# mirage/decompress

Measured on AMD Instinct MI355X. Metric: MiB/s inflate over N zlib streams (uncompressed bytes / wall second), higher is better.
Workload: dtype u8; 1 GPU; C2: 4096 x 256 KiB zlib streams per GPU, dynamic Huffman (libz level 6; even streams = slices of the reference's test/corpus, odd = order-2 Markov ASCII text, 64 symbols, seed 0xC2 + i, SURVEY 8(d)), Zl.Inf.Ns semantics, one stream per pair of wavefronts (decoder + copier); streams_per_gpu=4096, stream_bytes=262144, unique_streams=4096

## Files before the change

decompress_amd/csrc/inflate_wave.hip:

```cpp
#include <stdlib.h>
#include <string.h>
#include "inflate_util.hpp"

namespace md {
namespace wv {

constexpr uint32_t S = 264;
constexpr uint32_t SMIN = 48;
constexpr uint32_t KMAX = 64;
#ifndef MD_EMIT_SPLIT
#define MD_EMIT_SPLIT 1
#endif
#if defined(MD_DEBUG_KNOWN_BOUNDS)
#undef MD_EMIT_SPLIT
#define MD_EMIT_SPLIT 0
#endif
#ifndef MD_SPLIT_B
#define MD_SPLIT_B 4
#endif
#ifndef MD_RUNIN_NUM
#define MD_RUNIN_NUM 3
#define MD_RUNIN_DEN 2
#endif
constexpr uint32_t RUNIN_NUM = MD_RUNIN_NUM, RUNIN_DEN = MD_RUNIN_DEN;
constexpr uint32_t PASSES = 5;
constexpr uint32_t PASS_BITS = 1600, PASSES_MAX = 16;
#ifndef MD_RMAX
#define MD_RMAX 576
#endif
#ifndef MD_STAGE
#define MD_STAGE 5248
#endif
#ifndef MD_PAIR_OCC
#define MD_PAIR_OCC 5
#endif
constexpr uint32_t RMAX = MD_RMAX;
constexpr uint32_t STAGE = MD_STAGE;
constexpr uint32_t WIN_WORDS = 544;

constexpr uint32_t kLitSize = 852, kDistSize = 592;
constexpr uint32_t kLitRootMax = 512;
constexpr uint32_t kLitSubB = 0;
constexpr uint32_t kDistB = kLitSize - kLitRootMax;
constexpr uint32_t kLitB = kDistB + kDistSize;
constexpr uint32_t kStopEobI = kLitB + kLitRootMax;
constexpr uint32_t kStopBadI = kStopEobI + 2;
constexpr uint32_t kLutWords = kStopBadI + 2;
constexpr uint32_t kTbMask = 0xffe00000u;
constexpr uint32_t kLoopy = 0x100u;
static_assert(kDistB % 2 == 0 && kLitB % 2 == 0 && kStopEobI % 2 == 0 && kLutWords == 1448, "even table bases");
constexpr uint32_t kStEob = 100, kStTrunc = 101;
constexpr uint32_t kCountMatch = 1u << 20;
constexpr uint32_t kNearBit = 0x8000u;

struct Mail {
  uint32_t emitted;
  uint32_t copied;
  uint32_t kind;
  uint32_t total;
  uint32_t x;
  uint32_t stuck;
  uint32_t a, b;
};
constexpr uint32_t kJobRound = 0, kJobStored = 1, kJobQuit = 2, kJobEmit = 3;
constexpr uint32_t kHxUni = 4 * 64;
struct Smem {
  uint32_t win[WIN_WORDS];
  uint32_t lut[kLutWords];
  uint32_t mrec[RMAX];
  uint16_t mpos[RMAX];
  alignas(16) uint8_t stage[STAGE + 16];
  uint16_t list[RMAX];
  Mail mail;
};
struct HScratch {
  uint8_t lens[384];
  uint16_t work[320];
  uint32_t ctr;
};
#if MD_RMAX == 576 && MD_STAGE == 5248
static_assert(sizeof(Smem) <= 17920, "9 streams (18 wavefronts) per CU: 160 KiB / 9, in whole 512-byte units");
#endif
static_assert(RMAX % 64 == 0 && STAGE % 16 == 0 && RMAX * 2 >= (kHxUni + 6) * 4, "record rows, staging chunks, the emit job's words in `list`");
constexpr uint32_t kHScratchAt = 1136;
static_assert(kHScratchAt >= 4 + 572 + 8 && kHScratchAt % 16 == 0 && kHScratchAt + sizeof(HScratch) <= WIN_WORDS * 4, "header scratch lives behind the header's bits");
typedef MD_LDS Smem lds_smem;
typedef MD_LDS HScratch lds_hscratch;
__device__ __forceinline__ lds_hscratch *hscratch_of(lds_smem *sm) {
  return reinterpret_cast<lds_hscratch *>(reinterpret_cast<lds_u8 *>(sm->win) + kHScratchAt);
}

#ifdef MD_DEBUG_KNOWN_BOUNDS
constexpr uint32_t KB_ROUNDS = 512;
__device__ uint4 *g_kb_buf;
__device__ int g_kb_mode;
#endif
__device__ __forceinline__ uint32_t mk_entry(uint32_t n, uint32_t xb, uint32_t val8, uint32_t nbits, uint32_t tb) {
  return n | (xb << 5) | (val8 << 9) | (nbits << 17) | (tb << 21);
}
__device__ __forceinline__ uint32_t e_n(uint32_t e) { return e & 31; }
__device__ __forceinline__ uint32_t e_xb(uint32_t e) { return (e >> 5) & 15; }
__device__ __forceinline__ uint32_t e_val(uint32_t e) { return (e >> 9) & 255; }
__device__ __forceinline__ uint32_t e_tb(uint32_t e) { return e >> 21; }
__device__ __forceinline__ bool e_link(uint32_t e) { return e_tb(e) < kLitB && e_tb(e) != kDistB; }
__device__ __forceinline__ uint32_t e_root(uint32_t lroot) { return mk_entry(0, 0, 0, lroot, kLitB); }
__device__ __forceinline__ uint32_t lit_leaf(uint32_t sym, uint32_t codelen, uint32_t lroot, uint32_t droot) {
  if (sym < 256) return mk_entry(codelen, 0, sym, lroot, kLitB);
  if (sym == 256) return mk_entry(codelen, 0, 0, 0, kStopEobI);
  const uint32_t l = (sym - 257) & 31;
  const uint32_t xb = (l >= 8 && l < 28) ? (l - 4) >> 2 : 0;
  const uint32_t base3 = l < 8 ? l : l < 28 ? (4 + (l & 3)) << xb : l == 28 ? 255 : 0;
  return mk_entry(codelen + xb, xb, base3, droot, kDistB);
}
__device__ __forceinline__ uint32_t dist_leaf(uint32_t dv, uint32_t codelen, uint32_t lroot) {
  dv &= 31;
  if (dv >= 30) return mk_entry(codelen, 0, 0, 0, kStopBadI);
  const uint32_t xb = dv >= 4 ? (dv - 2) >> 1 : 0;
  const uint32_t m = dv < 4 ? dv : ((dv & 1) | 2);
  return mk_entry(codelen + xb, xb, m, lroot, kLitB);
}
__device__ __forceinline__ uint32_t dist_value(uint32_t m, uint32_t xb, uint32_t x) { return (m << xb) + 1 + x; }

struct Window {
  uint32_t w[8], wx;
  uint32_t base;
#ifdef MD_DEBUG_KNOWN_BOUNDS
  uint32_t kb_round, kb_sid;
#endif
  __device__ __forceinline__ void fetch(const uint8_t *__restrict__ body, uint32_t nbytes, uint32_t b, uint32_t lane) {
    base = b;
    const uint32_t off = b + lane * 32;
#pragma unroll
    for (int k = 0; k < 8; k++) w[k] = 0;
    if (off + 32 <= nbytes) __builtin_memcpy(w, body + off, 32);
    else if (off < nbytes)
      for (uint32_t k = 0; k < 32 && off + k < nbytes; k++) w[k >> 2] |= (uint32_t)body[off + k] << (8 * (k & 3));
    wx = 0;
    if (lane < WIN_WORDS - 512) {
      const uint32_t ox = b + 2048 + lane * 4;
      if (ox + 4 <= nbytes) __builtin_memcpy(&wx, body + ox, 4);
      else if (ox < nbytes)
        for (uint32_t k = 0; k < 4 && ox + k < nbytes; k++) wx |= (uint32_t)body[ox + k] << (8 * k);
    }
// ... 42 lines not shown
  __device__ __forceinline__ void drop(uint32_t k) {
    buf >>= k;
    n -= k;
  }
};

struct Canon {
  uint32_t cnt[16];
  uint32_t first[16];
  uint32_t offs[16];
  uint32_t max, min, root, left;
};
__device__ __forceinline__ uint32_t lane_rank(uint64_t m) {
  return __builtin_amdgcn_mbcnt_hi((uint32_t)(m >> 32), __builtin_amdgcn_mbcnt_lo((uint32_t)m, 0));
}
template <int K>
__device__ __forceinline__ void canon_counts(const uint32_t (&len)[K], uint32_t rootpref, Canon &c) {
#pragma unroll
  for (int l = 1; l < 16; l++) {
    uint32_t n = 0;
#pragma unroll
    for (int k = 0; k < K; k++) n += (uint32_t)__builtin_popcountll(__ballot(len[k] == (uint32_t)l));
    c.cnt[l] = n;
  }
  c.cnt[0] = 0;
  c.max = 0;
  c.min = 16;
#pragma unroll
  for (int l = 15; l >= 1; l--) {
    if (c.cnt[l] && c.max == 0) c.max = l;
    if (c.cnt[l]) c.min = l;
  }
  int left = 1;
  bool over = false;
  uint32_t code = 0, off = 0;
  c.first[0] = 0;
  c.offs[0] = 0;
#pragma unroll
  for (int l = 1; l < 16; l++) {
    left = (left << 1) - (int)c.cnt[l];
    over = over || left < 0;
    code = (code + c.cnt[l - 1]) << 1;
    c.first[l] = code;
    c.offs[l] = off;
    off += c.cnt[l];
  }
  c.left = over ? 0xffffffffu : (uint32_t)left;
  uint32_t root = rootpref;
  if (root > c.max) root = c.max;
  if (root < c.min) root = c.min;
  c.root = root;
}

template <int K, class LEAF>
__device__ __forceinline__ bool build_walk(const uint32_t (&len)[K], const Canon &c, lds_u32 *lut, uint32_t tb0, uint32_t sub0,
                                           uint32_t size, lds_hscratch *hs, uint32_t lane, uint32_t zero_entry, LEAF leaf) {
  const uint32_t root = c.root, rmask = (1u << root) - 1;
  uint32_t rev[K];
#pragma unroll
  for (int k = 0; k < K; k++) rev[k] = 0;
#pragma unroll
  for (int l = 1; l < 16; l++) {
    if (c.cnt[l]) {
      uint32_t base = 0;
#pragma unroll
      for (int k = 0; k < K; k++) {
        const uint64_t m = __ballot(len[k] == (uint32_t)l);
        if (len[k] == (uint32_t)l) {
          const uint32_t rank = base + lane_rank(m);
          rev[k] = __brev(c.first[l] + rank) >> (32 - l);
          hs->work[c.offs[l] + rank] = (uint16_t)(lane + 64 * k);
        }
        base += (uint32_t)__builtin_popcountll(m);
      }
    }
  }
  const uint32_t nroot = 1u << root;
  for (uint32_t i = lane; i < nroot; i += kWave) lut[tb0 + i] = 0;
  if (lane == 0) hs->ctr = 0;
  if (c.max > root) {
#pragma unroll
    for (int k = 0; k < K; k++)
      if (len[k] > root)
        __hip_atomic_fetch_max(&lut[tb0 + (rev[k] & rmask)], len[k], __ATOMIC_RELAXED, __HIP_MEMORY_SCOPE_WORKGROUP);
  }
  for (uint32_t i = lane; i < nroot; i += kWave) {
    const uint32_t v = lut[tb0 + i];
    uint32_t e;
    if (v) {
      const uint32_t sub = v - root;
      const uint32_t off = __hip_atomic_fetch_add(&hs->ctr, 1u << sub, __ATOMIC_RELAXED, __HIP_MEMORY_SCOPE_WORKGROUP);
      e = mk_entry(root, 0, 0, sub, (sub0 + off) & 2047);
    } else {
      const uint32_t cw = __brev(i) >> (32 - root);
      uint32_t fl = 0, ft = 0;
#pragma unroll
      for (int l = 15; l >= 1; l--) {
        if (c.cnt[l] && (uint32_t)l <= root) {
          const uint32_t t = (cw >> (root - l)) - c.first[l];
          if (t < c.cnt[l]) {
            fl = l;
            ft = c.offs[l] + t;
          }
        }
      }
      e = fl ? leaf((uint32_t)hs->work[ft], fl) : zero_entry;
    }
    lut[tb0 + i] = e;
  }
  const uint32_t used = nroot + uni(hs->ctr);
  if (used > size) return false;
  if (c.max > root) {
#pragma unroll
    for (int k = 0; k < K; k++) {
      if (len[k] > root) {
        const uint32_t link = lut[tb0 + (rev[k] & rmask)];
        const uint32_t sub = (link >> 17) & 15, tb = link >> 21;
        const uint32_t e = leaf(lane + 64 * k, len[k] - root);
        for (uint32_t j = rev[k] >> root; j < (1u << sub); j += 1u << (len[k] - root)) lut[tb + j] = e;
      }
    }
  }
  return true;
}

constexpr uint64_t kZig0 = 16ull | 17ull << 5 | 18ull << 10 | 0ull << 15 | 8ull << 20 | 7ull << 25 | 9ull << 30 | 6ull << 35 |
                           10ull << 40 | 5ull << 45 | 11ull << 50 | 4ull << 55;
constexpr uint64_t kZig1 = 12ull | 3ull << 5 | 13ull << 10 | 2ull << 15 | 14ull << 20 | 1ull << 25 | 15ull << 30;

template <class PF>
__device__ __noinline__ int dynamic_tables(lds_smem *sm, uint32_t bp_arg, uint32_t tot_arg, uint32_t lane, uint32_t *bp_out,
                                           uint32_t *lroot_out, PF &pf) {
  const uint32_t bp = uni(bp_arg), tot = uni(tot_arg);
  const lds_u32 *win = (const lds_u32 *)sm->win;
  lds_hscratch *hs = hscratch_of(sm);
  UBits ub;
  ub.init(win, bp);
  if ((int32_t)(tot - ub.pos()) < 14) return MD_UNEXPECTED_END_OF_INPUT;
  const uint32_t hlit = ub.peekb(5) + 257;
  ub.drop(5);
  const uint32_t hdist = ub.peekb(5) + 1;
  ub.drop(5);
  const uint32_t hclen = ub.peekb(4) + 4;
  ub.drop(4);
  uint32_t cl[1] = {0};
  for (uint32_t i = 0; i < hclen; i++) {
    ub.fill();
    if ((int32_t)(tot - ub.pos()) < 3) return MD_UNEXPECTED_END_OF_INPUT;
    const uint32_t v = ub.peekb(3);
    ub.drop(3);
    const uint32_t z = (uint32_t)((i < 12 ? kZig0 >> (5 * i) : kZig1 >> (5 * (i - 12))) & 31);
    if (lane == z) cl[0] = v;
  }
  Canon cc;
  canon_counts<1>(cl, 7, cc);
  uint32_t cmaxl, t_lo, t_hi;
  if (cc.max == 0) {
    cmaxl = 1;
    t_lo = lane == 0 ? (1u << 8) : 0xffffu;
    t_hi = 0xffffu;
  } else {
    if (cc.left != 0) return MD_INVALID_DICTIONARY;
    cmaxl = cc.max;
#pragma unroll
    for (int l = 1; l < 8; l++) {
      const uint64_t m = __ballot(cl[0] == (uint32_t)l);
      if (cl[0] == (uint32_t)l) hs->work[cc.offs[l] + lane_rank(m)] = (uint16_t)lane;
    }
    uint32_t t[2];
#pragma unroll
    for (int h = 0; h < 2; h++) {
      const uint32_t i = lane + 64 * h;
      const uint32_t cw = __brev(i & ((1u << cmaxl) - 1)) >> (32 - cmaxl);
      uint32_t fl = 0, ft = 0;
#pragma unroll
      for (int l = 7; l >= 1; l--) {
        if (cc.cnt[l] && (uint32_t)l <= cmaxl) {
          const uint32_t x = (cw >> (cmaxl - l)) - cc.first[l];
          if (x < cc.cnt[l]) {
            fl = l;
            ft = cc.offs[l] + x;
          }
        }
      }
      t[h] = fl ? ((uint32_t)hs->work[ft] | (fl << 8)) : 0xffffu;
// ... 4 lines not shown
  const uint32_t max_res = hlit + hdist;
  for (uint32_t x = lane; x < 384; x += kWave) hs->lens[x] = 0;
  auto run_lengths = [&](auto checked) -> int {
    constexpr bool CHECK = decltype(checked)::value;
    uint32_t i = 0, prev = 0;
    while (i < max_res) {
      ub.fill();
      if (CHECK && (int32_t)(tot - ub.pos()) < (int32_t)cmaxl) return MD_UNEXPECTED_END_OF_INPUT;
      const uint32_t idx = ub.peekb(cmaxl);
      const uint32_t e_lo = __builtin_amdgcn_readlane(t_lo, idx & 63), e_hi = __builtin_amdgcn_readlane(t_hi, idx & 63);
      const uint32_t e = idx < 64 ? e_lo : e_hi;
      if (e == 0xffffu) return MD_INVALID_DICTIONARY;
      const uint32_t sym = e & 0xff;
      ub.drop(e >> 8);
      if (sym < 16) {
        hs->lens[i] = (uint8_t)sym;
        prev = sym;
        i++;
      } else {
        const uint32_t nb = sym == 16 ? 2 : sym == 17 ? 3 : 7;
        if (sym == 16 && i == 0) return MD_INVALID_DICTIONARY;
        ub.fill();
        if (CHECK && (int32_t)(tot - ub.pos()) < (int32_t)nb) return MD_UNEXPECTED_END_OF_INPUT;
        const uint32_t copy = ub.peekb(nb) + (sym == 18 ? 11 : 3);
        ub.drop(nb);
        const uint32_t val = sym == 16 ? prev : 0;
        if (i + copy > max_res) return MD_INVALID_DICTIONARY;
        if (val)
          for (uint32_t x = lane; x < copy; x += kWave) hs->lens[i + x] = (uint8_t)val;
        prev = val;
        i += copy;
      }
    }
    return MD_OK;
  };
  {
    const bool plenty = (int32_t)(tot - ub.pos()) >= 316 * 14 + 64;
    const int rc = plenty ? run_lengths(std::false_type{}) : run_lengths(std::true_type{});
    if (rc != MD_OK) return rc;
  }
  *bp_out = ub.pos();
  pf.tick_lds(P_HDR_LENS);
  if (uni(hs->lens[256]) == 0) return MD_INVALID_DICTIONARY;
  uint32_t ll[5], dl[1];
#pragma unroll
  for (int k = 0; k < 5; k++) ll[k] = lane + 64 * k < hlit ? (uint32_t)hs->lens[lane + 64 * k] : 0u;
  dl[0] = lane < hdist ? (uint32_t)hs->lens[hlit + lane] : 0u;
  Canon cl_, cd_;
  canon_counts<5>(ll, 9, cl_);
  canon_counts<1>(dl, 6, cd_);
  if (cl_.left == 0xffffffffu || (cl_.left > 0 && cl_.max != 1)) return MD_INVALID_DICTIONARY;
  const uint32_t lroot = cl_.root;
  uint32_t droot;
  lds_u32 *lut = (lds_u32 *)sm->lut;
  if (cd_.max == 0) {
    droot = 1;
  } else {
    if (cd_.left == 0xffffffffu || (cd_.left > 0 && cd_.max != 1)) return MD_INVALID_DICTIONARY;
    droot = cd_.root;
  }
  if (!build_walk<5>(ll, cl_, lut, kLitB, kLitSubB, kLitSize, hs, lane, e_root(lroot),
                     [=](uint32_t sym, uint32_t codelen) { return lit_leaf(sym, codelen, lroot, droot); }))
    return MD_INVALID_DICTIONARY;
  pf.tick_lds(P_HDR_LIT);
  if (cd_.max == 0) {
    if (lane == 0) {
      lut[kDistB] = dist_leaf(0, 1, lroot);
      lut[kDistB + 1] = mk_entry(0, 0, 0, 0, kStopBadI);
    }
  } else if (!build_walk<1>(dl, cd_, lut, kDistB, kDistB + (1u << droot), kDistSize, hs, lane, e_root(lroot),
                            [=](uint32_t sym, uint32_t codelen) { return dist_leaf(sym, codelen, lroot); }))
    return MD_INVALID_DICTIONARY;
  const bool loopy = cl_.left > 0 || (cd_.max != 0 && cd_.left > 0);
  *lroot_out = lroot | (loopy ? kLoopy : 0u);
  return MD_OK;
}

__device__ __noinline__ void fixed_tables(lds_smem *sm, uint32_t lane, uint32_t *lroot_out) {
  lds_hscratch *hs = hscratch_of(sm);
  uint32_t ll[5], dl[1];
#pragma unroll
  for (int k = 0; k < 5; k++) {
    const uint32_t n = lane + 64 * k;
    ll[k] = n < 144 ? 8 : n < 256 ? 9 : n < 280 ? 7 : n < 288 ? 8 : 0;
  }
  dl[0] = lane < 32 ? 5 : 0;
  Canon cl_, cd_;
  canon_counts<5>(ll, 9, cl_);
  canon_counts<1>(dl, 6, cd_);
  const uint32_t lroot = cl_.root, droot = cd_.root;
  lds_u32 *lut = (lds_u32 *)sm->lut;
  build_walk<5>(ll, cl_, lut, kLitB, kLitSubB, kLitSize, hs, lane, e_root(lroot),
                [=](uint32_t sym, uint32_t codelen) { return lit_leaf(sym, codelen, lroot, droot); });
  build_walk<1>(dl, cd_, lut, kDistB, kDistB + (1u << droot), kDistSize, hs, lane, e_root(lroot),
                [=](uint32_t sym, uint32_t codelen) { return dist_leaf(sym, codelen, lroot); });
  *lroot_out = lroot;
}

struct Cursor {
  uint32_t w0, w1, w2, wa;
  __device__ __forceinline__ void init(const lds_u32 *win, uint32_t p) {
    wa = (p >> 5) << 2;
    const lds_u32 *q = reinterpret_cast<const lds_u32 *>(reinterpret_cast<const lds_u8 *>(win) + wa);
    w0 = q[0];
    w1 = q[1];
    w2 = q[2];
  }
  __device__ __forceinline__ uint32_t peek(uint32_t p) const { return __builtin_amdgcn_alignbit(w1, w0, p); }
  __device__ __forceinline__ void seek(const lds_u32 *win, uint32_t pn) {
    const uint32_t wan = (pn >> 5) << 2;
    const bool ge = wan != wa;
    w0 = ge ? w1 : w0;
    w1 = ge ? w2 : w1;
    wa = wan;
    w2 = *reinterpret_cast<const lds_u32 *>(reinterpret_cast<const lds_u8 *>(win) + wa + 8);
  }
};
__device__ __forceinline__ uint32_t lut_step(const lds_u32 *lut, uint32_t e, uint32_t w) {
  return lut_at(lut, e >> 21, __builtin_amdgcn_ubfe(w, 0, e >> 17));
}

template <bool COUNT, bool BUDGET, bool MID = false>
__device__ __forceinline__ void sync_pass(const lds_u32 *win, const lds_u32 *lut, uint32_t lroot, bool go, uint32_t start,
                                          uint32_t limit, uint32_t &end, uint32_t &stop, uint32_t &nb, uint32_t mthr = 0,
                                          uint32_t *midp = nullptr, uint32_t *midcnt = nullptr) {
  if (go) {
    uint32_t p = start, e = e_root(lroot), cnt = 0;
    uint32_t mp = 0xffffffffu, mc = 0;
    bool got = false;
    if (MID && start >= mthr) {
      mp = start;
      got = true;
    }
    if (p < limit) {
      const uint32_t thr = (kLitB << 21) | limit;
      uint32_t slot = 0, key;
      Cursor c;
      c.init(win, start);
      do {
        const uint32_t w = c.peek(p);
        const uint32_t en = lut_step(lut, e, w);
        const uint32_t n = e_n(en);
        if (COUNT) {
          const uint32_t xb = e_xb(en);
          const uint32_t len1 = e_val(en) + __builtin_amdgcn_ubfe(w, n - xb, xb) + (kCountMatch + 2);
          cnt += (e_tb(en) == kLitB ? 1u : 0u) + (e_tb(en) == kDistB ? len1 : 0u);
        }
        p += n;
// ... 369 lines not shown
    const uint32_t n = ml - skip;
    const bool fast = d >= n && n <= 32;
    const uint32_t qb = todo ? qs + skip : 0xffffffffu, qe = todo ? qs + ml : 0xffffffffu;
    uint32_t jlo = 0, jhi = 0;
#pragma unroll
    for (uint32_t st = 32; st > 0; st >>= 1) {
      const uint32_t ve = __shfl(qe, jlo + st - 1), vb = __shfl(qb, jhi + st - 1);
      jlo = ve <= sa ? jlo + st : jlo;
      jhi = vb < sb ? jhi + st : jhi;
    }
    jhi = jhi < lane ? jhi : lane;
    uint64_t need = 0;
    if (sa < sb && jlo < jhi) need = ((jhi >= 64 ? 0ull : (1ull << jhi)) - 1ull) & ~((1ull << jlo) - 1ull);
    uint64_t done = 0;
    pf.tick_lds(P_NEAR_LOAD);
    for (uint32_t guard = 0; __ballot(todo) != 0; guard++) {
      if (guard > kWave) {
        *stuck = true;
        return;
      }
      pf.count(C_NEAR_IT);
      const bool ready = todo && (need & ~done) == 0;
      if constexpr (PF::on) {
        if (__ballot(ready && !fast)) pf.count(C_LONG_NEAR);
      }
      pf.tick_lds(P_NEAR);
      if (ready && fast) {
        lds_u8 *dd = stage + qs + skip;
        const lds_u8 *ss = stage + sa;
        const uint64_t v0 = lds_ld64(ss), v1 = lds_ld64(ss + 8), v2 = lds_ld64(ss + 16), v3 = lds_ld64(ss + 24);
        lds_put(dd, v0, n < 8 ? n : 8);
        if (n > 8) lds_put(dd + 8, v1, n < 16 ? n - 8 : 8);
        if (n > 16) {
          lds_put(dd + 16, v2, n < 24 ? n - 16 : 8);
          if (n > 24) lds_put(dd + 24, v3, n - 24);
        }
      }
      pf.tick_lds(P_NEAR_FAST);
      for (uint64_t lm = __ballot(ready && !fast); lm; lm &= lm - 1) {
        const uint32_t l = (uint32_t)__builtin_ctzll(lm);
        wave_copy(stage, rdlane(qs + skip, l), rdlane(sa, l), rdlane(n, l), rdlane(d, l), lane);
      }
      pf.tick_lds(P_NEAR_SLOW);
      done |= __ballot(ready);
      todo = todo && !ready;
      pf.tick_lds(P_NEAR_UPD);
    }
  }
  pf.tick(P_NEAR);
}

template <class PF>
__device__ __forceinline__ void copy_round(lds_smem *sm, Sink &sk, uint32_t lane, uint32_t total, uint32_t nrec, bool *stuck, PF &pf) {
  const lds_u32 *mrec = (const lds_u32 *)sm->mrec;
  const lds_u16 *mpos = (const lds_u16 *)sm->mpos;
  lds_u16 *list = (lds_u16 *)sm->list;
  const uint32_t R0 = sk.pos, rb = sk.sbase();
  uint32_t nnear = 0;
#ifdef MD_DEBUG_KNOWN_BOUNDS
  {
    const int kbm = __builtin_amdgcn_readfirstlane(g_kb_mode);
    if (kbm & 8) {
      sk.pos += total;
      return;
    }
    if (kbm & 4) {
      sk.flush(total);
      return;
    }
  }
#endif
  __builtin_amdgcn_fence(__ATOMIC_RELEASE, "workgroup");
  if (R0 + 40 > sk.cap) {
    copy_far_guarded<PF>(mrec, mpos, list, sk.stage, sk.g, R0, rb, sk.cap, lane, nrec, &nnear);
    pf.tick(P_FAR);
  } else {
    copy_far(mrec, mpos, list, sk, lane, nrec, &nnear, pf);
  }
  copy_near_all(mrec, mpos, list, sk, lane, nnear, stuck, pf);
  sk.flush(total);
  pf.tick(P_ADLER);
}

__device__ __forceinline__ uint32_t mail_ld(const MD_LDS uint32_t *p) {
  return __hip_atomic_load(p, __ATOMIC_RELAXED, __HIP_MEMORY_SCOPE_WORKGROUP);
}
__device__ __forceinline__ void mail_st(MD_LDS uint32_t *p, uint32_t v) {
  __hip_atomic_store(p, v, __ATOMIC_RELAXED, __HIP_MEMORY_SCOPE_WORKGROUP);
}
__device__ __forceinline__ bool mail_wait_idle(lds_smem *sm, uint32_t sent) {
  while (uni(mail_ld(&sm->mail.copied)) != sent) __builtin_amdgcn_s_sleep(2);
  asm volatile("" ::: "memory");
  return uni(mail_ld(&sm->mail.stuck)) == 0;
}
__device__ __forceinline__ void mail_post(lds_smem *sm, uint32_t lane, uint32_t kind, uint32_t total, uint32_t x, uint32_t &sent) {
  if (lane == 0) {
    sm->mail.kind = kind;
    sm->mail.total = total;
    sm->mail.x = x;
  }
  asm volatile("s_waitcnt lgkmcnt(0)" ::: "memory");
  sent++;
  if (lane == 0) mail_st(&sm->mail.emitted, sent);
}

template <class PF, bool PAIR, bool BUDGET>
__device__ __forceinline__ int inflate_block(lds_smem *sm, const uint8_t *__restrict__ body, uint32_t body_len, Sink &sk,
                                             uint32_t lroot, uint32_t lane, uint32_t *bp_io, uint32_t *zone_io, Window &wnd,
                                             uint32_t &sent, PF &pf) {
  uint32_t bp = *bp_io;
  lds_u32 *win = (lds_u32 *)sm->win;
  const lds_u32 *lut = (const lds_u32 *)sm->lut;
  lds_u32 *mrec = (lds_u32 *)sm->mrec;
  lds_u16 *mpos = (lds_u16 *)sm->mpos;
  const uint32_t total_bits = body_len * 8;
  uint32_t zs = *zone_io;
  constexpr bool kSplit = PAIR && !BUDGET && MD_EMIT_SPLIT != 0;
  for (;;) {
    const uint32_t base = (bp >> 5) << 2;
    wnd.ensure(win, body, body_len, base, lane);
    const uint32_t rbp = bp - base * 8, tot = total_bits - base * 8;
    pf.tick(P_ENSURE);
    pf.count(C_ROUNDS);
    pf.count(C_PASSES);
    uint32_t start = rbp + lane * zs, end = 0, stop = 0, nb = 0;
    uint32_t midp = 0xffffffffu, midcnt = 0;
    const uint32_t limit = rbp + (lane + 1) * zs;
    const uint32_t runin_ = (zs * RUNIN_NUM) / RUNIN_DEN, runin = runin_ < lane * zs ? runin_ : lane * zs;
    bool counted = false;
#ifdef MD_DEBUG_KNOWN_BOUNDS
    const int kbm = __builtin_amdgcn_readfirstlane(g_kb_mode);
    const bool kb_can = wnd.kb_round < KB_ROUNDS;
    uint4 *kbp = g_kb_buf + ((size_t)wnd.kb_sid * KB_ROUNDS + wnd.kb_round) * kWave + lane;
    wnd.kb_round++;
    if ((kbm & 3) == 2 && kb_can) {
      const uint4 v = *kbp;
      start = v.x;
      end = v.y;
      stop = v.z & 0xffffu;
      counted = (v.z >> 16) != 0;
      nb = v.w;
    } else {
#endif
    sync_pass<false, BUDGET>(win, lut, lroot, true, start - runin, limit, end, stop, nb);
    pf.tick(P_DECODE1);
    const uint32_t passes = zs * PASSES >= PASS_BITS ? PASSES : PASS_BITS / zs > PASSES_MAX ? PASSES_MAX : PASS_BITS / zs;
    for (uint32_t it = 0; it < passes; it++) {
      const uint32_t pe = wave_shr1(end), ps = wave_shr1(stop);
      const bool redo = lane == 0 ? !counted : (ps == 0 && (pe != start || !counted));
      if (__ballot(redo) == 0) break;
      if (redo && lane > 0) start = pe;
      pf.count(C_PASSES);
      if constexpr (kSplit) sync_pass<true, BUDGET, true>(win, lut, lroot, redo, start, limit, end, stop, nb, limit - (zs * MD_SPLIT_B) / 8, &midp, &midcnt);
      else sync_pass<true, BUDGET>(win, lut, lroot, redo, start, limit, end, stop, nb);
      counted = counted || redo;
    }
#ifdef MD_DEBUG_KNOWN_BOUNDS
      if ((kbm & 3) == 1 && kb_can) *kbp = make_uint4(start, end, stop | (counted ? 0x10000u : 0u), nb);
    }
#endif
    pf.tick(P_DECODE2);
    uint32_t nvalid;
    {
      const uint32_t pe = wave_shr1(end), ps = wave_shr1(stop);
      const uint64_t bad = __ballot(!counted || (lane > 0 && (ps != 0 || pe != start)));
      nvalid = bad ? (uint32_t)__builtin_ctzll(bad) : 64;
    }
    const uint32_t R0 = sk.pos, rb = sk.sbase();
    uint32_t mynb = lane < nvalid ? nb : 0;
    const uint32_t off = wave_excl_scan(mynb, lane);
    if (nvalid < 64) pf.count(C_END_CHAIN);
    {
      const uint32_t bend = ((off + mynb) & (kCountMatch - 1)), rend = (off + mynb) >> 20;
      const uint64_t fits = __ballot((R0 - rb) + bend <= STAGE - 16 && rend <= RMAX);
      const uint32_t nfit = fits == ~0ull ? 64 : (uint32_t)__builtin_ctzll(~fits);
      if (nfit < nvalid) {
        pf.count(rdlane(rend, nfit) > RMAX ? C_END_RECORDS : C_END_FIT);
        nvalid = nfit ? nfit : 1;
      }
    }
    const bool mine = lane < nvalid;
    if (!mine) mynb = 0;
    const uint32_t boff = off & (kCountMatch - 1), roff = off >> 20;
    const uint32_t q0 = R0 + boff;
    LaneOut lo;
    lo.endp = end;
    lo.stopc = 0;
    lo.bytes = 0;
    lo.nm = 0;
    if constexpr (PAIR) {
      pf.tick(P_DECODE2);
      if (!mail_wait_idle(sm, sent)) return MD_E_HIP;
      pf.tick(P_WAIT_DEC);
    }
    bool split = false;
    uint32_t bq = 0, br = 0;
    LaneOut lob;
    lob.endp = 0, lob.stopc = 0, lob.bytes = 0, lob.nm = 0;
    bool gob = false;
    if constexpr (kSplit) split = zs >= 128;
    {
      const uint32_t all = rdlane(off + mynb, nvalid - 1) & (kCountMatch - 1);
      const bool plain = tot >= rbp + kWave * zs + 64 && R0 >= 32768u && all <= sk.cap - R0 && (R0 - rb) + all <= STAGE - 16;
      uint32_t alimit = limit;
      if constexpr (kSplit) {
        if (split) {
          gob = mine && midp != 0xffffffffu && midp < limit && midp >= start;
          bq = midcnt & (kCountMatch - 1);
          br = midcnt >> 20;
          lds_u32 *hx = reinterpret_cast<lds_u32 *>(sm->list);
          hx[4 * lane + 0] = gob ? midp : 0xffffffffu;
          hx[4 * lane + 1] = limit;
          hx[4 * lane + 2] = q0 + bq;
          hx[4 * lane + 3] = roff + br;
          if (lane < 6) hx[kHxUni + lane] = lane == 0 ? lroot : lane == 1 ? tot : lane == 2 ? rb : lane == 3 ? R0 : lane == 4 ? sk.cap : (plain ? 0u : 1u);
          mail_post(sm, lane, kJobEmit, 0, 0, sent);
          alimit = gob ? midp : limit;
        }
      }
      if (plain && !BUDGET) emit_pass<false, false>(win, lut, lroot, mrec, mpos, sk.stage, roff, tot, mine, start, alimit, q0, rb, R0, sk.cap, lo);
      else emit_pass<true, BUDGET>(win, lut, lroot, mrec, mpos, sk.stage, roff, tot, mine, start, alimit, q0, rb, R0, sk.cap, lo);
      if constexpr (kSplit) {
        if (split) {
          if (!mail_wait_idle(sm, sent)) return MD_E_HIP;
          const lds_u32 *hx = reinterpret_cast<const lds_u32 *>(sm->list);
          if (gob) {
            lob.endp = hx[4 * lane + 0];
            lob.stopc = hx[4 * lane + 1];
            lob.bytes = hx[4 * lane + 2];
            lob.nm = hx[4 * lane + 3];
// ... 36 lines not shown
    } else {
      copy_round(sm, sk, lane, total, nrec, &stuck, pf);
    }
    pf.count(C_LANES, nvalid);
    if (stuck || (nbp == bp && total == 0 && (lstop == 0 || lstop == kStTrunc))) return MD_E_HIP;
    {
      const uint32_t bits = nbp - bp;
      const uint64_t want = (uint64_t)(STAGE - STAGE / 8) * bits / ((uint64_t)kWave * (total ? total : 1u));
      zs = want > S ? S : want < SMIN ? SMIN : (uint32_t)want;
    }
    bp = nbp;
    if (lstop == kStEob) break;
    if (lstop != 0 && lstop != kStTrunc) return (int)lstop;
  }
  *bp_io = bp;
  *zone_io = zs;
  return MD_OK;
}

__device__ __forceinline__ void copy_stored(Sink &sk, const uint8_t *__restrict__ body, uint32_t p, uint32_t len, uint32_t lane) {
  const uint8_t *q = body + p;
  uint32_t left = len;
  while (left) {
    const uint32_t seg = left < STAGE - 16 ? left : STAGE - 16;
    const uint32_t s0 = sk.pos - sk.sbase();
    for (uint32_t j = lane; j < seg; j += kWave) sk.stage[s0 + j] = q[j];
    sk.flush(seg);
    q += seg;
    left -= seg;
  }
}

template <class PF>
__device__ __forceinline__ void copier_main(lds_smem *sm, const uint8_t *__restrict__ body, Sink &sk, uint32_t lane, PF &pf) {
  uint32_t done = 0;
  for (;;) {
    while (uni(mail_ld(&sm->mail.emitted)) == done) __builtin_amdgcn_s_sleep(2);
    asm volatile("" ::: "memory");
    const uint32_t kind = uni(sm->mail.kind), total = uni(sm->mail.total), x = uni(sm->mail.x);
    pf.tick(P_WAIT_COPY);
    if (kind == kJobQuit) break;
    bool stuck = false;
    if (kind == kJobRound) copy_round(sm, sk, lane, total, x, &stuck, pf);
    else if (kind == kJobEmit) {
      if constexpr (MD_EMIT_SPLIT != 0) {
        lds_u32 *hx = reinterpret_cast<lds_u32 *>(sm->list);
        const uint32_t bstart = hx[4 * lane + 0], blimit = hx[4 * lane + 1], bq0 = hx[4 * lane + 2], brec = hx[4 * lane + 3];
        const uint32_t lroot = uni(hx[kHxUni + 0]), tot = uni(hx[kHxUni + 1]), rb = uni(hx[kHxUni + 2]), R0 = uni(hx[kHxUni + 3]),
                       cap = uni(hx[kHxUni + 4]), checked = uni(hx[kHxUni + 5]);
        const bool go = bstart != 0xffffffffu;
        LaneOut lo;
        lo.endp = bstart, lo.stopc = 0, lo.bytes = 0, lo.nm = 0;
        const lds_u32 *win = (const lds_u32 *)sm->win;
        const lds_u32 *lut = (const lds_u32 *)sm->lut;
        if (checked) emit_pass<true, false>(win, lut, lroot, (lds_u32 *)sm->mrec, (lds_u16 *)sm->mpos, sk.stage, brec, tot, go, go ? bstart : 0u, blimit, bq0, rb, R0, cap, lo);
        else emit_pass<false, false>(win, lut, lroot, (lds_u32 *)sm->mrec, (lds_u16 *)sm->mpos, sk.stage, brec, tot, go, go ? bstart : 0u, blimit, bq0, rb, R0, cap, lo);
        hx[4 * lane + 0] = lo.endp;
        hx[4 * lane + 1] = lo.stopc;
        hx[4 * lane + 2] = lo.bytes;
        hx[4 * lane + 3] = lo.nm;
      }
    } else copy_stored(sk, body, x, total, lane);
    if (lane == 0) {
      sm->mail.a = sk.a;
      sm->mail.b = sk.b;
      if (stuck) sm->mail.stuck = 1;
    }
    asm volatile("s_waitcnt lgkmcnt(0)" ::: "memory");
    done++;
    if (lane == 0) mail_st(&sm->mail.copied, done);
  }
}

struct Cont {
  const uint32_t *start_bit, *hist_len, *adler_in;
  uint64_t *resume_bits, *resume_out;
  uint32_t *resume_adler, *resume_last;
};

template <bool PROF, bool PAIR>
__global__ __launch_bounds__(PAIR ? 2 * kWave : kWave, PAIR ? MD_PAIR_OCC : 2) void inflate_wave_kernel(
    int format, uint32_t n, const uint8_t *__restrict__ in, const uint64_t *__restrict__ in_off,
    const uint64_t *__restrict__ in_len, uint8_t *out, const uint64_t *__restrict__ out_off,
    const uint64_t *__restrict__ out_cap, uint64_t *__restrict__ out_len,
    uint64_t *__restrict__ consumed, int32_t *__restrict__ status, uint32_t *__restrict__ checksum,
    uint64_t *__restrict__ dbg, const uint32_t *__restrict__ order, Cont cont) {
  __shared__ Smem smem;
  lds_smem *sm = (lds_smem *)&smem;
  Prof<PROF> pf;
  pf.init();
  const uint32_t lane = threadIdx.x & (kWave - 1);
  const uint32_t wave = PAIR ? uni(threadIdx.x / kWave) : 0u;
  if (blockIdx.x >= n) return;
  const uint32_t sid = order ? order[blockIdx.x] : blockIdx.x;

  const uint8_t *src = in + in_off[sid];
  uint64_t slen64 = in_len[sid], cap64 = out_cap[sid];
  if (slen64 > MD_MAX_INFLATE_IN) {
    if (threadIdx.x == 0) {
      out_len[sid] = 0;
      consumed[sid] = 0;
      status[sid] = MD_E_INVALID_ARGUMENT;
      if (checksum) checksum[sid] = 0;
    }
    return;
  }
  const uint32_t slen = (uint32_t)slen64;
  const bool cap_clamped = cap64 > MD_MAX_STREAM;
  const uint32_t cap = cap_clamped ? (uint32_t)MD_MAX_STREAM : (uint32_t)cap64;

  int rc = MD_OK;
  uint32_t body_off = 0, body_len = slen;
  if (format == MD_FORMAT_ZLIB) {
    if (slen < 2) rc = MD_UNEXPECTED_END_OF_INPUT;
    else {
      uint32_t cmf = src[0], flg = src[1];
      if (((cmf << 8) + flg) % 31 != 0 || (cmf & 0xf) != 8) rc = MD_INVALID_HEADER;
      else if (slen < 6) rc = MD_UNEXPECTED_END_OF_INPUT;
      else {
        body_off = 2;
        body_len = slen - 6;
      }
    }
  }
  const uint8_t *body = src + body_off;

  Sink sk;
  sk.stage = (lds_u8 *)sm->stage;
  sk.g = out + out_off[sid];
  sk.cap = cap;
  const uint32_t hist = cont.hist_len ? cont.hist_len[sid] : 0u, adler0 = cont.adler_in ? cont.adler_in[sid] : 1u;
  sk.pos = hist < cap ? hist : cap;
  sk.lane = lane;
  sk.a = adler0 & 0xffffu;
  sk.b = adler0 >> 16;
  sk.want_adler = (checksum != nullptr) || format == MD_FORMAT_ZLIB || cont.resume_adler != nullptr;

  if (threadIdx.x < 4) sm->lut[kStopEobI + threadIdx.x] = mk_entry(0, 0, 0, 0, kStopEobI + (threadIdx.x & 2));
  if constexpr (PAIR) {
    if (threadIdx.x < sizeof(Mail) / 4) ((lds_u32 *)&sm->mail)[threadIdx.x] = threadIdx.x == 6 ? sk.a : threadIdx.x == 7 ? sk.b : 0u;
    __syncthreads();
    if (wave == 1) {
      copier_main(sm, body, sk, lane, pf);
      if constexpr (PROF) {
        if (lane == 0 && sid == 0 && dbg) {
          const int mine[] = {P_FAR, P_NEAR, P_ADLER, P_NEAR_FAST, P_NEAR_SLOW, P_NEAR_UPD, P_NEAR_LOAD, P_FAR_REC, P_FAR_LOAD, P_WAIT_COPY};
          for (int i : mine) dbg[i] = pf.acc[i];
          dbg[P_COUNT + C_NEAR_IT] = pf.cnt[C_NEAR_IT];
          dbg[P_COUNT + C_LONG_NEAR] = pf.cnt[C_LONG_NEAR];
          dbg[P_COUNT + C_FAR_SPILL] = pf.cnt[C_FAR_SPILL];
        }
      }
      return;
    }
  }

  lds_u32 *win = (lds_u32 *)sm->win;
  const uint32_t total_bits = body_len * 8;
  uint32_t bp = cont.start_bit ? cont.start_bit[sid] & 7u : 0u;
  uint32_t zone = S;
  uint32_t sent = 0;
  uint32_t fixed_lroot = 0;
  Window wnd;
  wnd.base = 0xffffffffu;
#ifdef MD_DEBUG_KNOWN_BOUNDS
  wnd.kb_round = 0;
  wnd.kb_sid = sid;
#endif
  if (cont.resume_bits && lane == 0) {
    cont.resume_bits[sid] = bp;
    cont.resume_out[sid] = sk.pos;
    cont.resume_adler[sid] = adler0;
    cont.resume_last[sid] = 0;
  }

  if (rc == MD_OK) {
    bool last = false;
    uint32_t lds_base = 0xffffffffu;
    while (!last && rc == MD_OK) {
      uint32_t base = (bp >> 5) << 2;
      if (lds_base != 0xffffffffu && bp >= lds_base * 8 && bp - lds_base * 8 <= 4096) base = lds_base;
      else {
        wnd.ensure(win, body, body_len, base, lane);
        lds_base = base;
      }
      uint32_t rbp = bp - base * 8;
      const uint32_t tot = total_bits - base * 8;
      if ((int32_t)(tot - rbp) < 3) {
        rc = MD_UNEXPECTED_END_OF_INPUT;
        break;
      }
// ... 9 lines not shown
          rbp += 7;
          bp += 7;
          block_done = true;
          if (last || rbp + 3 > tot) break;
          const uint32_t h = uni(peek(win, rbp)) & 7u;
          if (((h >> 1) & 3) != 1) break;
          last = h & 1;
          rbp += 3;
          bp += 3;
          block_done = false;
        }
      }
      if (block_done) {
      } else if (type == 0) {
        uint32_t p = (bp + 7) >> 3;
        if (body_len - p < 4) {
          rc = MD_UNEXPECTED_END_OF_INPUT;
          break;
        }
        uint32_t h4;
        if (p + 4 <= base + (WIN_WORDS - 2) * 4) h4 = uni(peek(win, (p - base) * 8));
        else h4 = (uint32_t)body[p] | ((uint32_t)body[p + 1] << 8) | ((uint32_t)body[p + 2] << 16) | ((uint32_t)body[p + 3] << 24);
        uint32_t len = h4 & 0xffff, nlen = h4 >> 16;
        p += 4;
        if (nlen != 0xffff - len) rc = MD_INVALID_COMPLEMENT_OF_LENGTH;
        else if (len > body_len - p) rc = MD_UNEXPECTED_END_OF_INPUT;
        else if (len > sk.cap - sk.pos) rc = MD_UNEXPECTED_END_OF_OUTPUT;
        else {
          if (len) {
            if constexpr (PAIR) {
              if (!mail_wait_idle(sm, sent)) rc = MD_E_HIP;
              mail_post(sm, lane, kJobStored, len, p, sent);
              sk.pos += len;
            } else {
              copy_stored(sk, body, p, len, lane);
            }
          }
          p += len;
          bp = p * 8;
        }
      } else if (type == 3) {
        rc = MD_INVALID_KIND_OF_BLOCK;
      } else {
        uint32_t lroot = 0;
        if (type == 1) {
          if (fixed_lroot == 0) {
            fixed_tables(sm, lane, &lroot);
            fixed_lroot = uni(lroot);
          }
          lroot = fixed_lroot;
        } else {
          uint32_t hend = 0;
          fixed_lroot = 0;
          rc = dynamic_tables(sm, rbp, tot, lane, &hend, &lroot, pf);
          bp = base * 8 + hend;
        }
        lroot = uni(lroot);
        pf.tick(P_HEADER);
        if (rc == MD_OK) {
          if (lroot & kLoopy) rc = inflate_block<Prof<PROF>, PAIR, true>(sm, body, body_len, sk, lroot & 15, lane, &bp, &zone, wnd, sent, pf);
          else rc = inflate_block<Prof<PROF>, PAIR, false>(sm, body, body_len, sk, lroot, lane, &bp, &zone, wnd, sent, pf);
          lds_base = 0xffffffffu;
        }
      }
      if (cont.resume_bits && rc == MD_OK) {
        if constexpr (PAIR) {
          if (!mail_wait_idle(sm, sent)) rc = MD_E_HIP;
          sk.a = uni(sm->mail.a);
          sk.b = uni(sm->mail.b);
        }
        if (lane == 0) {
          cont.resume_bits[sid] = bp;
          cont.resume_out[sid] = sk.pos;
          cont.resume_adler[sid] = (sk.b << 16) | sk.a;
          cont.resume_last[sid] = last ? 1u : 0u;
        }
      }
    }
  }
  if constexpr (PAIR) {
    if (!mail_wait_idle(sm, sent) && rc == MD_OK) rc = MD_E_HIP;
    sk.a = uni(sm->mail.a);
    sk.b = uni(sm->mail.b);
    mail_post(sm, lane, kJobQuit, 0, 0, sent);
  }
  uint32_t used = (bp + 7) >> 3;
  uint32_t adler = (sk.b << 16) | sk.a;
  if (rc == MD_OK && format == MD_FORMAT_ZLIB) {
    const uint8_t *t = src + 2 + used;
    uint32_t want = ((uint32_t)t[0] << 24) | ((uint32_t)t[1] << 16) | ((uint32_t)t[2] << 8) | t[3];
    if (want != adler) rc = MD_INVALID_CHECKSUM;
    used += 6;
  }
  if (rc == MD_UNEXPECTED_END_OF_OUTPUT && cap_clamped) rc = MD_E_INVALID_ARGUMENT;
  if (lane == 0) {
    out_len[sid] = sk.pos;
    consumed[sid] = rc == MD_OK ? used : 0;
    status[sid] = rc;
    if (checksum) checksum[sid] = adler;
  }
  if constexpr (PROF) {
    if (lane == 0 && sid == 0 && dbg) {
      if constexpr (PAIR) {
        const int mine[] = {P_ENSURE, P_DECODE1, P_DECODE2, P_EMIT_A, P_HEADER, P_HDR_LENS, P_HDR_LIT, P_WAIT_DEC};
        for (int i : mine) dbg[i] = pf.acc[i];
        for (int i = 0; i < C_COUNT; i++)
          if (i != C_NEAR_IT && i != C_LONG_NEAR && i != C_FAR_SPILL) dbg[P_COUNT + i] = pf.cnt[i];
      } else {
        for (int i = 0; i < P_COUNT; i++) dbg[i] = pf.acc[i];
        for (int i = 0; i < C_COUNT; i++) dbg[P_COUNT + i] = pf.cnt[i];
      }
    }
  }
}
// ... 103 lines not shown
```

Measured before the change: 248,900 MiB/s.

## Overlap Huffman sub-tables with match-record pool to fit ten streams per CU

Shrinks the per-stream LDS footprint by sizing the LUT for typical sub-table use and letting rare oversized sub-tables borrow the tail of the match-record array. Sub-tables are now allocated downward from the distance root, and a returned per-block record cap limits how many records a round may produce when borrowing happens. The goal is to raise occupancy from 9 to 10 stream pairs per CU. In exchange, the decoder must wait for the copier to go idle before overwriting borrowed records, and the record budget per round can shrink for unusual code tables.

Result: no change. 248,300 MiB/s, median of 3 (-0.2%).

```diff
diff --git a/decompress_amd/csrc/inflate_wave.hip b/decompress_amd/csrc/inflate_wave.hip
--- a/decompress_amd/csrc/inflate_wave.hip
+++ b/decompress_amd/csrc/inflate_wave.hip
@@ -40,15 +40,23 @@
 
 constexpr uint32_t kLitSize = 852, kDistSize = 592;
 constexpr uint32_t kLitRootMax = 512;
-constexpr uint32_t kLitSubB = 0;
-constexpr uint32_t kDistB = kLitSize - kLitRootMax;
-constexpr uint32_t kLitB = kDistB + kDistSize;
+constexpr uint32_t kDistRootMax = 64;
+#ifndef MD_LUT_WORDS
+#define MD_LUT_WORDS 1076
+#endif
+constexpr uint32_t kLutOwn = MD_LUT_WORDS;
+constexpr uint32_t kSubRoom = kLutOwn - 4 - kLitRootMax - kDistRootMax;
+constexpr uint32_t kSubMax = (kLitSize - kLitRootMax) + (kDistSize - kDistRootMax);
+constexpr uint32_t kBorrow = kSubMax > kSubRoom ? kSubMax - kSubRoom : 0;
+constexpr uint32_t kDistB = kBorrow + kSubRoom;
+constexpr uint32_t kLitB = kDistB + kDistRootMax;
 constexpr uint32_t kStopEobI = kLitB + kLitRootMax;
 constexpr uint32_t kStopBadI = kStopEobI + 2;
 constexpr uint32_t kLutWords = kStopBadI + 2;
 constexpr uint32_t kTbMask = 0xffe00000u;
 constexpr uint32_t kLoopy = 0x100u;
-static_assert(kDistB % 2 == 0 && kLitB % 2 == 0 && kStopEobI % 2 == 0 && kLutWords == 1448, "even table bases");
+static_assert(kDistB % 2 == 0 && kLitB % 2 == 0 && kStopEobI % 2 == 0 && kBorrow % 2 == 0 && kLutWords == kBorrow + kLutOwn, "even table bases");
+static_assert(kSubRoom >= kLitSize - kLitRootMax && kLutWords <= 2048, "lit/len sub-tables always fit the room; an 11-bit tb");
 constexpr uint32_t kStEob = 100, kStTrunc = 101;
 constexpr uint32_t kCountMatch = 1u << 20;
 constexpr uint32_t kNearBit = 0x8000u;
@@ -66,8 +74,7 @@
 constexpr uint32_t kHxUni = 4 * 64;
 struct Smem {
   uint32_t win[WIN_WORDS];
-  uint32_t lut[kLutWords];
-  uint32_t mrec[RMAX];
+  uint32_t rl[RMAX + kLutOwn];
   uint16_t mpos[RMAX];
   alignas(16) uint8_t stage[STAGE + 16];
   uint16_t list[RMAX];
@@ -78,9 +85,10 @@
   uint16_t work[320];
   uint32_t ctr;
 };
-#if MD_RMAX == 576 && MD_STAGE == 5248
-static_assert(sizeof(Smem) <= 17920, "9 streams (18 wavefronts) per CU: 160 KiB / 9, in whole 512-byte units");
+#if MD_RMAX == 576 && MD_STAGE == 5248 && MD_LUT_WORDS == 1076
+static_assert(sizeof(Smem) <= 16384, "10 streams (20 wavefronts) per CU: 160 KiB / 10, in whole 512-byte units");
 #endif
+static_assert(RMAX >= kBorrow + S / 2 + 1, "the smallest record pool");
 static_assert(RMAX % 64 == 0 && STAGE % 16 == 0 && RMAX * 2 >= (kHxUni + 6) * 4, "record rows, staging chunks, the emit job's words in `list`");
 constexpr uint32_t kHScratchAt = 1136;
 static_assert(kHScratchAt >= 4 + 572 + 8 && kHScratchAt % 16 == 0 && kHScratchAt + sizeof(HScratch) <= WIN_WORDS * 4, "header scratch lives behind the header's bits");
@@ -89,6 +97,8 @@
 __device__ __forceinline__ lds_hscratch *hscratch_of(lds_smem *sm) {
   return reinterpret_cast<lds_hscratch *>(reinterpret_cast<lds_u8 *>(sm->win) + kHScratchAt);
 }
+__device__ __forceinline__ lds_u32 *mrec_of(lds_smem *sm) { return (lds_u32 *)sm->rl; }
+__device__ __forceinline__ lds_u32 *lut_of(lds_smem *sm) { return (lds_u32 *)sm->rl + (RMAX - kBorrow); }
 
 #ifdef MD_DEBUG_KNOWN_BOUNDS
 constexpr uint32_t KB_ROUNDS = 512;
@@ -237,9 +247,9 @@
   c.root = root;
 }
 
-template <int K, class LEAF>
-__device__ __forceinline__ bool build_walk(const uint32_t (&len)[K], const Canon &c, lds_u32 *lut, uint32_t tb0, uint32_t sub0,
-                                           uint32_t size, lds_hscratch *hs, uint32_t lane, uint32_t zero_entry, LEAF leaf) {
+template <int K, class LEAF, class ROOM>
+__device__ __forceinline__ int build_walk(const uint32_t (&len)[K], const Canon &c, lds_u32 *lut, uint32_t tb0, uint32_t &top,
+                                          uint32_t size, lds_hscratch *hs, uint32_t lane, uint32_t zero_entry, LEAF leaf, ROOM room) {
   const uint32_t root = c.root, rmask = (1u << root) - 1;
   uint32_t rev[K];
 #pragma unroll
@@ -275,7 +285,7 @@
     if (v) {
       const uint32_t sub = v - root;
       const uint32_t off = __hip_atomic_fetch_add(&hs->ctr, 1u << sub, __ATOMIC_RELAXED, __HIP_MEMORY_SCOPE_WORKGROUP);
-      e = mk_entry(root, 0, 0, sub, (sub0 + off) & 2047);
+      e = mk_entry(root, 0, 0, sub, (top - off - (1u << sub)) & 2047);
     } else {
       const uint32_t cw = __brev(i) >> (32 - root);
       uint32_t fl = 0, ft = 0;
@@ -293,8 +303,10 @@
     }
     lut[tb0 + i] = e;
   }
-  const uint32_t used = nroot + uni(hs->ctr);
-  if (used > size) return false;
+  const uint32_t nsub = uni(hs->ctr), used = nroot + nsub;
+  if (used > size) return MD_INVALID_DICTIONARY;
+  top -= nsub;
+  if (!room(top)) return MD_E_HIP;
   if (c.max > root) {
 #pragma unroll
     for (int k = 0; k < K; k++) {
@@ -306,16 +318,18 @@
       }
     }
   }
-  return true;
+  return MD_OK;
 }
 
 constexpr uint64_t kZig0 = 16ull | 17ull << 5 | 18ull << 10 | 0ull << 15 | 8ull << 20 | 7ull << 25 | 9ull << 30 | 6ull << 35 |
                            10ull << 40 | 5ull << 45 | 11ull << 50 | 4ull << 55;
 constexpr uint64_t kZig1 = 12ull | 3ull << 5 | 13ull << 10 | 2ull << 15 | 14ull << 20 | 1ull << 25 | 15ull << 30;
 
-template <class PF>
-__device__ __noinline__ int dynamic_tables(lds_smem *sm, uint32_t bp_arg, uint32_t tot_arg, uint32_t lane, uint32_t *bp_out,
-                                           uint32_t *lroot_out, PF &pf) {
+__device__ __forceinline__ bool mail_wait_idle(lds_smem *sm, uint32_t sent);
+
+template <class PF, bool PAIR>
+__device__ __noinline__ int dynamic_tables(lds_smem *sm, uint32_t bp_arg, uint32_t tot_arg, uint32_t sent_arg, uint32_t lane,
+                                           uint32_t *bp_out, uint32_t *lroot_out, PF &pf) {
   const uint32_t bp = uni(bp_arg), tot = uni(tot_arg);
   const lds_u32 *win = (const lds_u32 *)sm->win;
   lds_hscratch *hs = hscratch_of(sm);
@@ -426,27 +440,38 @@
   if (cl_.left == 0xffffffffu || (cl_.left > 0 && cl_.max != 1)) return MD_INVALID_DICTIONARY;
   const uint32_t lroot = cl_.root;
   uint32_t droot;
-  lds_u32 *lut = (lds_u32 *)sm->lut;
+  lds_u32 *lut = lut_of(sm);
   if (cd_.max == 0) {
     droot = 1;
   } else {
     if (cd_.left == 0xffffffffu || (cd_.left > 0 && cd_.max != 1)) return MD_INVALID_DICTIONARY;
     droot = cd_.root;
   }
-  if (!build_walk<5>(ll, cl_, lut, kLitB, kLitSubB, kLitSize, hs, lane, e_root(lroot),
-                     [=](uint32_t sym, uint32_t codelen) { return lit_leaf(sym, codelen, lroot, droot); }))
-    return MD_INVALID_DICTIONARY;
+  const uint32_t sent = uni(sent_arg);
+  bool idle = false;
+  const auto room = [&](uint32_t lo) {
+    if (!PAIR || lo >= kBorrow || idle) return true;
+    idle = true;
+    return mail_wait_idle(sm, sent);
+  };
+  uint32_t top = kDistB;
+  int rc = build_walk<5>(ll, cl_, lut, kLitB, top, kLitSize, hs, lane, e_root(lroot),
+                         [=](uint32_t sym, uint32_t codelen) { return lit_leaf(sym, codelen, lroot, droot); }, room);
+  if (rc != MD_OK) return rc;
   pf.tick_lds(P_HDR_LIT);
   if (cd_.max == 0) {
     if (lane == 0) {
       lut[kDistB] = dist_leaf(0, 1, lroot);
       lut[kDistB + 1] = mk_entry(0, 0, 0, 0, kStopBadI);
     }
-  } else if (!build_walk<1>(dl, cd_, lut, kDistB, kDistB + (1u << droot), kDistSize, hs, lane, e_root(lroot),
-                            [=](uint32_t sym, uint32_t codelen) { return dist_leaf(sym, codelen, lroot); }))
-    return MD_INVALID_DICTIONARY;
+  } else {
+    rc = build_walk<1>(dl, cd_, lut, kDistB, top, kDistSize, hs, lane, e_root(lroot),
+                       [=](uint32_t sym, uint32_t codelen) { return dist_leaf(sym, codelen, lroot); }, room);
+    if (rc != MD_OK) return rc;
+  }
   const bool loopy = cl_.left > 0 || (cd_.max != 0 && cd_.left > 0);
-  *lroot_out = lroot | (loopy ? kLoopy : 0u);
+  const uint32_t rcap = top >= kBorrow ? RMAX : RMAX - (kBorrow - top);
+  *lroot_out = lroot | (loopy ? kLoopy : 0u) | (rcap << 16);
   return MD_OK;
 }
 
@@ -463,11 +488,13 @@
   canon_counts<5>(ll, 9, cl_);
   canon_counts<1>(dl, 6, cd_);
   const uint32_t lroot = cl_.root, droot = cd_.root;
-  lds_u32 *lut = (lds_u32 *)sm->lut;
-  build_walk<5>(ll, cl_, lut, kLitB, kLitSubB, kLitSize, hs, lane, e_root(lroot),
-                [=](uint32_t sym, uint32_t codelen) { return lit_leaf(sym, codelen, lroot, droot); });
-  build_walk<1>(dl, cd_, lut, kDistB, kDistB + (1u << droot), kDistSize, hs, lane, e_root(lroot),
-                [=](uint32_t sym, uint32_t codelen) { return dist_leaf(sym, codelen, lroot); });
+  lds_u32 *lut = lut_of(sm);
+  uint32_t top = kDistB;
+  const auto room = [](uint32_t) { return true; };
+  build_walk<5>(ll, cl_, lut, kLitB, top, kLitSize, hs, lane, e_root(lroot),
+                [=](uint32_t sym, uint32_t codelen) { return lit_leaf(sym, codelen, lroot, droot); }, room);
+  build_walk<1>(dl, cd_, lut, kDistB, top, kDistSize, hs, lane, e_root(lroot),
+                [=](uint32_t sym, uint32_t codelen) { return dist_leaf(sym, codelen, lroot); }, room);
   *lroot_out = lroot;
 }
 
@@ -943,7 +970,7 @@
 
 template <class PF>
 __device__ __forceinline__ void copy_round(lds_smem *sm, Sink &sk, uint32_t lane, uint32_t total, uint32_t nrec, bool *stuck, PF &pf) {
-  const lds_u32 *mrec = (const lds_u32 *)sm->mrec;
+  const lds_u32 *mrec = mrec_of(sm);
   const lds_u16 *mpos = (const lds_u16 *)sm->mpos;
   lds_u16 *list = (lds_u16 *)sm->list;
   const uint32_t R0 = sk.pos, rb = sk.sbase();
@@ -997,12 +1024,12 @@
 
 template <class PF, bool PAIR, bool BUDGET>
 __device__ __forceinline__ int inflate_block(lds_smem *sm, const uint8_t *__restrict__ body, uint32_t body_len, Sink &sk,
-                                             uint32_t lroot, uint32_t lane, uint32_t *bp_io, uint32_t *zone_io, Window &wnd,
-                                             uint32_t &sent, PF &pf) {
+                                             uint32_t lroot, uint32_t rcap, uint32_t lane, uint32_t *bp_io, uint32_t *zone_io,
+                                             Window &wnd, uint32_t &sent, PF &pf) {
   uint32_t bp = *bp_io;
   lds_u32 *win = (lds_u32 *)sm->win;
-  const lds_u32 *lut = (const lds_u32 *)sm->lut;
-  lds_u32 *mrec = (lds_u32 *)sm->mrec;
+  const lds_u32 *lut = lut_of(sm);
+  lds_u32 *mrec = mrec_of(sm);
   lds_u16 *mpos = (lds_u16 *)sm->mpos;
   const uint32_t total_bits = body_len * 8;
   uint32_t zs = *zone_io;
@@ -1063,10 +1090,10 @@
     if (nvalid < 64) pf.count(C_END_CHAIN);
     {
       const uint32_t bend = ((off + mynb) & (kCountMatch - 1)), rend = (off + mynb) >> 20;
-      const uint64_t fits = __ballot((R0 - rb) + bend <= STAGE - 16 && rend <= RMAX);
+      const uint64_t fits = __ballot((R0 - rb) + bend <= STAGE - 16 && rend <= rcap);
       const uint32_t nfit = fits == ~0ull ? 64 : (uint32_t)__builtin_ctzll(~fits);
       if (nfit < nvalid) {
-        pf.count(rdlane(rend, nfit) > RMAX ? C_END_RECORDS : C_END_FIT);
+        pf.count(rdlane(rend, nfit) > rcap ? C_END_RECORDS : C_END_FIT);
         nvalid = nfit ? nfit : 1;
       }
     }
@@ -1209,9 +1236,9 @@
         LaneOut lo;
         lo.endp = bstart, lo.stopc = 0, lo.bytes = 0, lo.nm = 0;
         const lds_u32 *win = (const lds_u32 *)sm->win;
-        const lds_u32 *lut = (const lds_u32 *)sm->lut;
-        if (checked) emit_pass<true, false>(win, lut, lroot, (lds_u32 *)sm->mrec, (lds_u16 *)sm->mpos, sk.stage, brec, tot, go, go ? bstart : 0u, blimit, bq0, rb, R0, cap, lo);
-        else emit_pass<false, false>(win, lut, lroot, (lds_u32 *)sm->mrec, (lds_u16 *)sm->mpos, sk.stage, brec, tot, go, go ? bstart : 0u, blimit, bq0, rb, R0, cap, lo);
+        const lds_u32 *lut = lut_of(sm);
+        if (checked) emit_pass<true, false>(win, lut, lroot, mrec_of(sm), (lds_u16 *)sm->mpos, sk.stage, brec, tot, go, go ? bstart : 0u, blimit, bq0, rb, R0, cap, lo);
+        else emit_pass<false, false>(win, lut, lroot, mrec_of(sm), (lds_u16 *)sm->mpos, sk.stage, brec, tot, go, go ? bstart : 0u, blimit, bq0, rb, R0, cap, lo);
         hx[4 * lane + 0] = lo.endp;
         hx[4 * lane + 1] = lo.stopc;
         hx[4 * lane + 2] = lo.bytes;
@@ -1293,7 +1320,7 @@
   sk.b = adler0 >> 16;
   sk.want_adler = (checksum != nullptr) || format == MD_FORMAT_ZLIB || cont.resume_adler != nullptr;
 
-  if (threadIdx.x < 4) sm->lut[kStopEobI + threadIdx.x] = mk_entry(0, 0, 0, 0, kStopEobI + (threadIdx.x & 2));
+  if (threadIdx.x < 4) lut_of(sm)[kStopEobI + threadIdx.x] = mk_entry(0, 0, 0, 0, kStopEobI + (threadIdx.x & 2));
   if constexpr (PAIR) {
     if (threadIdx.x < sizeof(Mail) / 4) ((lds_u32 *)&sm->mail)[threadIdx.x] = threadIdx.x == 6 ? sk.a : threadIdx.x == 7 ? sk.b : 0u;
     __syncthreads();
@@ -1409,14 +1436,16 @@
         } else {
           uint32_t hend = 0;
           fixed_lroot = 0;
-          rc = dynamic_tables(sm, rbp, tot, lane, &hend, &lroot, pf);
+          rc = dynamic_tables<Prof<PROF>, PAIR>(sm, rbp, tot, sent, lane, &hend, &lroot, pf);
           bp = base * 8 + hend;
         }
         lroot = uni(lroot);
         pf.tick(P_HEADER);
         if (rc == MD_OK) {
-          if (lroot & kLoopy) rc = inflate_block<Prof<PROF>, PAIR, true>(sm, body, body_len, sk, lroot & 15, lane, &bp, &zone, wnd, sent, pf);
-          else rc = inflate_block<Prof<PROF>, PAIR, false>(sm, body, body_len, sk, lroot, lane, &bp, &zone, wnd, sent, pf);
+          const uint32_t rcap = type == 1 ? RMAX : lroot >> 16;
+          lroot &= 0xffffu;
+          if (lroot & kLoopy) rc = inflate_block<Prof<PROF>, PAIR, true>(sm, body, body_len, sk, lroot & 15, rcap, lane, &bp, &zone, wnd, sent, pf);
+          else rc = inflate_block<Prof<PROF>, PAIR, false>(sm, body, body_len, sk, lroot, rcap, lane, &bp, &zone, wnd, sent, pf);
           lds_base = 0xffffffffu;
         }
       }
```
